# g1mv/density

Measured on AMD Instinct MI355X. Metric: MB/s encode+decode (round-trip) per GPU + compression ratio, dickens/enwik8, higher is better.
Workload: dtype u32

## Files before the change

### density_amd/csrc/api.hip

```cpp
#include "api_internal.hpp"

namespace density {
namespace api {

thread_local std::string g_last_error;
int g_profiling = 0;
int g_variant = 0;
uint64_t g_pass_decodes = 0;
uint64_t g_stream_stats[4] = {0, 0, 0, 0};
DeviceCtx g_ctx[kMaxDevices];

void set_error(const char* what, hipError_t e) {
    g_last_error = what;
    if (e != hipSuccess) { g_last_error += ": "; g_last_error += hipGetErrorString(e); }
}

DeviceCtx* acquire_ctx() {
    int dev = -1;
    hipError_t e = hipGetDevice(&dev);
    if (e != hipSuccess || dev < 0 || dev >= kMaxDevices) { set_error("no HIP device available", e); return nullptr; }
    DeviceCtx* c = &g_ctx[dev];
    std::lock_guard<std::mutex> lk(c->mu);
    if (!c->ready) {
        hipDeviceProp_t prop;
// ... 139 lines not shown
                         uint8_t* ws, hipStream_t s, density_hip_header_t* header_out, Form form) {
    const EncodePlan p = plan_encode(algo, n, chunk);
    if (p.n_chunks > 0xffffffffull) { set_error("too many chunks"); return DENSITY_HIP_ERR_ARGUMENT; }
    form = settle_form(form, algo, d_in, n, chunk, p.n_chunks);
    const size_t bound = form == Form::Paged ? container_bound_paged(algo, n, chunk) : form == Form::Slotted ? container_bound_slotted(algo, n, chunk) : container_bound(algo, n, chunk);
    if (cap < bound) { set_error("output capacity below density_hip_container_bound()"); return DENSITY_HIP_ERR_CAPACITY; }
    const uint32_t nch = (uint32_t)p.n_chunks;
    uint32_t* d_err = p.err(ws);
    uint64_t* d_sizes = p.sizes(ws);
    const density_hip_header_t hdr = make_header(algo, chunk, nch, n, (want_index(algo) ? DENSITY_HIP_FLAG_BLOCK_INDEX : 0) |
                                                 (form == Form::Slotted ? DENSITY_HIP_FLAG_SLOTTED : form == Form::Paged ? DENSITY_HIP_FLAG_PAGED : 0));
    const bool with_index = hdr.flags & DENSITY_HIP_FLAG_BLOCK_INDEX;
    const uint64_t pbase = payload_base(nch, n, with_index);
    uint8_t* d_index = with_index ? d_out + index_base(nch) : nullptr;
    Profiler prof(c, s);
    hipError_t e = hipMemsetAsync(d_err, 0, sizeof(uint32_t), s);
    if (e != hipSuccess) { set_error("hipMemsetAsync", e); return DENSITY_HIP_ERR_RUNTIME; }
    if (form == Form::Paged) {
        const uint64_t dir_base = paged_dir_base(nch, n), pages_base = paged_pages_base(nch, n, chunk);
        const uint32_t ppc = paged_pages_per_chunk(chunk);
        uint32_t* d_counter = p.page_counter(ws);
        e = hipMemsetAsync(d_counter, 0, sizeof(uint32_t), s);
        if (e == hipSuccess) e = launch_rotor_encode_paged(d_in, n, chunk, nch, d_out + pages_base, (uint32_t)std::min<uint64_t>((cap - pages_base) / kPageBytes, 0xffffu),
                                                         d_counter, reinterpret_cast<uint32_t*>(d_out + dir_base), page_dir_words(ppc), d_sizes, d_index, d_err, s);
        prof.mark(encode_kernel_name(algo));
        if (e == hipSuccess) e = launch_layout_encode_paged(d_sizes, nch, hdr, dir_base, dir_base + paged_dir_bytes(nch, chunk), pages_base, d_out, cap, d_counter, d_err, s);
        prof.mark("layout_encode");
    } else if (nch == 1 || form == Form::Slotted) {
        const uint64_t stride = nch == 1 ? 0 : p.stride;
        e = codec_encode(algo, d_in, n, chunk, nch, d_out + pbase, stride, d_sizes, d_index, p.tables(ws), p.zmap(ws), p.stage(ws), d_err, s);
        prof.mark(encode_kernel_name(algo));
        if (e == hipSuccess) e = launch_layout_encode(d_sizes, nch, hdr, pbase, d_out, cap, p.offsets(ws), d_err, s, stride);
        prof.mark("layout_encode");
    } else {
        constexpr uint32_t kStitchBatches = 4;
        uint32_t per = nch, batches = 1;
        if (algo == DENSITY_HIP_CHAMELEON && nch >= 512 && variant(kVarBatchedStitch)) {
            batches = nch / 256 < kStitchBatches ? nch / 256 : kStitchBatches;
            per = ((nch + batches - 1) / batches + 255) / 256 * 256;
            batches = (nch + per - 1) / per;
        }
        for (uint32_t k = 0; k < batches && e == hipSuccess; ++k) {
// ... 33 lines not shown
    const DecodePlan p = plan_decode(h.algo, h.n_chunks, h.chunk_size);
    uint32_t* d_err = p.err(ws);
    uint64_t *d_sizes = p.sizes(ws), *d_offsets = p.offsets(ws), *d_produced = p.produced(ws);
    uint32_t* d_zmap = p.zmap(ws);
    Profiler prof(c, s);
    hipError_t e = hipMemsetAsync(d_err, 0, sizeof(uint32_t), s);
    const bool with_index = h.flags & DENSITY_HIP_FLAG_BLOCK_INDEX;
    const uint8_t* d_index = with_index ? d_in + index_base(h.n_chunks) : nullptr;
    const size_t trailer = header_trailer(h), body_len = h.container_len - trailer;
    if (trailer) container_size = body_len;
    if (h.flags & DENSITY_HIP_FLAG_PAGED) {
        const size_t dir_base = paged_dir_base(h.n_chunks, h.total_len), pages_base = paged_pages_base(h.n_chunks, h.total_len, h.chunk_size);
        if (g_rotor_unsafe || !rotor_decode_eligible(d_out, h.n_chunks, h.chunk_size, h.total_len, d_index, d_zmap) || (uintptr_t)(d_in + pages_base) % 4 != 0) {
            set_error("a paged container needs the rotation decoder (chunks of at most 4 MiB, 4-byte aligned buffers)"); return DENSITY_HIP_ERR_UNSUPPORTED;
        }
        if (e == hipSuccess) e = launch_layout_decode_paged(d_in, h.n_chunks, d_sizes, d_offsets, s);
        prof.mark("layout_decode");
        if (e == hipSuccess) e = launch_rotor_decode_paged(d_in + pages_base, d_offsets, d_sizes, h.n_chunks, d_out, h.chunk_size, h.total_len, d_index,
                                                         reinterpret_cast<const uint32_t*>(d_in + dir_base), page_dir_words(paged_pages_per_chunk(h.chunk_size)),
                                                         (uint32_t)((body_len - pages_base) / kPageBytes), d_zmap, d_produced, d_err, s);
        prof.mark(decode_kernel_name(h.algo));
    } else {
        if (e == hipSuccess) e = launch_layout_decode(d_in, container_size, h.n_chunks, payload_base(h.n_chunks, h.total_len, with_index), d_sizes, d_offsets, d_err, s,
                                                      (h.flags & DENSITY_HIP_FLAG_SLOTTED) ? slot_stride(h.algo, h.chunk_size) : 0);
        prof.mark("layout_decode");
        if (e == hipSuccess) e = codec_decode(h.algo, d_in, d_offsets, d_sizes, h.n_chunks, d_out, h.chunk_size, h.total_len, true, d_index, d_produced, d_err, p.tables(ws), d_zmap, s,
                                              p.pass(ws, ws_size));
        prof.mark(decode_kernel_name(h.algo));
    }
    if (trailer) {
        if (e == hipSuccess) e = launch_checksum(d_out, h.total_len, h.chunk_size, h.n_chunks, reinterpret_cast<uint32_t*>(d_produced), d_in + body_len, d_err, s);
        prof.mark("checksum_verify");
    }
// ... 346 lines not shown
```

### density_amd/csrc/api_internal.hpp

```cpp
#pragma once
#include <hip/hip_runtime.h>

#include <algorithm>
#include <cstdio>
#include <cstring>
#include <initializer_list>
#include <mutex>
#include <string>
#include <vector>

#include "../../include/density_hip.h"
#include "kernels.hpp"

namespace density {
namespace api {

constexpr int kMaxDevices = 16;
constexpr size_t kAlign = 256;
constexpr size_t kMaxChunk = 1u << 30;

extern thread_local std::string g_last_error;
extern int g_profiling;
extern int g_variant;
extern uint64_t g_pass_decodes;
// ... 195 lines not shown
constexpr size_t kSerialTableBudget = 8ull << 30;
inline size_t serial_slots(int algo, size_t n_chunks) {
    if (algo == DENSITY_HIP_CHAMELEON) return 0;
    const size_t by_memory = kSerialTableBudget / serial_table_bytes(algo);
    size_t cap = kSerialSlots < by_memory ? kSerialSlots : by_memory;
    if (const char* e = debug_env("DENSITY_HIP_SERIAL_SLOTS")) { const size_t v = (size_t)atoll(e); if (v >= 1 && v < cap) cap = v; }
    return n_chunks < cap ? n_chunks : cap;
}
inline size_t serial_tables(int algo, size_t n_chunks) { return algo == DENSITY_HIP_CHAMELEON ? 0 : align_up(serial_slots(algo, n_chunks) * serial_table_bytes(algo), kAlign); }

inline size_t zmap_bytes(int algo, size_t n_chunks) { return (algo == DENSITY_HIP_CHAMELEON && n_chunks <= kMaxPipelinedChunks) ? align_up((n_chunks ? n_chunks : 1) * kZmapWordsPerChunk * 4, kAlign) : 0; }

struct EncodePlan {
    size_t chunk, n_chunks, stride, off_err, off_sizes, off_offsets, off_slots, off_tables, off_zmap, off_stage, total;
    uint32_t* err(uint8_t* ws) const { return reinterpret_cast<uint32_t*>(ws + off_err); }
    uint32_t* page_counter(uint8_t* ws) const { return err(ws) + 4; }
    uint64_t* sizes(uint8_t* ws) const { return reinterpret_cast<uint64_t*>(ws + off_sizes); }
    uint64_t* offsets(uint8_t* ws) const { return reinterpret_cast<uint64_t*>(ws + off_offsets); }
    uint64_t* carry(uint8_t* ws) const { return offsets(ws) + n_chunks; }
    uint8_t* slots(uint8_t* ws) const { return ws + off_slots; }
    uint8_t* tables(uint8_t* ws) const { return ws + off_tables; }
    uint32_t* zmap(uint8_t* ws) const { return off_stage > off_zmap ? reinterpret_cast<uint32_t*>(ws + off_zmap) : nullptr; }
    uint8_t* stage(uint8_t* ws) const { return total > off_stage ? ws + off_stage : nullptr; }
};
EncodePlan plan_encode(int algo, size_t n, size_t chunk);
struct DecodePlan {
    size_t off_err, off_sizes, off_offsets, off_produced, off_tables, off_zmap, off_pass, total, total_with_passes;
    uint32_t* err(uint8_t* ws) const { return reinterpret_cast<uint32_t*>(ws + off_err); }
    uint32_t* damaged(uint8_t* ws) const { return err(ws) + 1; }
    uint64_t* sizes(uint8_t* ws) const { return reinterpret_cast<uint64_t*>(ws + off_sizes); }
    uint64_t* offsets(uint8_t* ws) const { return reinterpret_cast<uint64_t*>(ws + off_offsets); }
// ... 40 lines not shown
```

### density_amd/csrc/container.hip

```cpp
#include "common.hpp"
#include "kernels.hpp"

namespace density {

namespace {

constexpr uint32_t kScanThreads = 1024;
constexpr uint32_t kHeaderBytes = 32;
static_assert(sizeof(density_hip_header_t) == kHeaderBytes, "container header is 32 bytes");

__device__ __forceinline__ uint64_t align16(uint64_t v) { return (v + 15ull) & ~15ull; }

__device__ __forceinline__ uint64_t block_inclusive_scan(uint64_t v, uint64_t* wave_sums , uint64_t* total) {
    const uint32_t lane = threadIdx.x & 63u, wave = threadIdx.x >> 6;
#pragma unroll
    for (int d = 1; d < 64; d <<= 1) {
        const uint32_t lo = bperm(lane >= (uint32_t)d ? lane - d : lane, (uint32_t)v);
        const uint32_t hi = bperm(lane >= (uint32_t)d ? lane - d : lane, (uint32_t)(v >> 32));
        if (lane >= (uint32_t)d) v += ((uint64_t)hi << 32) | lo;
    }
    if (lane == 63) wave_sums[wave] = v;
    __syncthreads();
    uint64_t prefix = 0, sum = 0;
    for (uint32_t i = 0; i < kScanThreads / 64; ++i) {
// ... 69 lines not shown
        *carry = end_scratch;
        if (is_last) {
            hdr.container_len = end_scratch;
            *reinterpret_cast<density_hip_header_t*>(container) = hdr;
        }
        if (end_scratch > capacity) atomicOr(err, 2u);
    }
    if (is_first) {
        const uint64_t table_end = kHeaderBytes + 4ull * hdr.n_chunks, ibase = (table_end + 15) / 16 * 16;
        const uint64_t iend = ibase + ((hdr.flags & DENSITY_HIP_FLAG_BLOCK_INDEX) ? (hdr.total_len + 255) / 256 : 0);
        if (threadIdx.x < ibase - table_end) container[table_end + threadIdx.x] = 0;
        if (threadIdx.x >= 32 && threadIdx.x - 32 < base - iend && base <= capacity) container[iend + threadIdx.x - 32] = 0;
    }
}

__global__ __launch_bounds__(kScanThreads) void layout_encode_paged_kernel(const uint64_t* __restrict__ sizes, uint32_t n, density_hip_header_t hdr, uint64_t dir_base,
                                                                           uint64_t dir_end, uint64_t pages_base, uint8_t* __restrict__ container, uint64_t capacity,
                                                                           const uint32_t* __restrict__ page_counter, uint32_t* __restrict__ err) {
    uint32_t* table = reinterpret_cast<uint32_t*>(container + kHeaderBytes);
    for (uint32_t i = threadIdx.x; i < n; i += kScanThreads) table[i] = (uint32_t)sizes[i];
    if (threadIdx.x == 0) {
        hdr.container_len = pages_base + (uint64_t)*page_counter * kPageBytes;
        *reinterpret_cast<density_hip_header_t*>(container) = hdr;
        if (hdr.container_len > capacity) atomicOr(err, 2u);
    }
    const uint64_t table_end = kHeaderBytes + 4ull * n, ibase = (table_end + 15) / 16 * 16;
    const uint64_t iend = ibase + (hdr.total_len + 255) / 256;
    if (threadIdx.x < ibase - table_end) container[table_end + threadIdx.x] = 0;
    if (threadIdx.x >= 32 && threadIdx.x - 32 < dir_base - iend) container[iend + threadIdx.x - 32] = 0;
    for (uint64_t i = dir_end + threadIdx.x; i < pages_base; i += kScanThreads) container[i] = 0;
}
__global__ __launch_bounds__(256) void clear_directory_tails_kernel(uint32_t n, uint64_t dir_base, uint64_t dir_end, uint8_t* __restrict__ container) {
    const uint32_t c = blockIdx.x * 4u + (threadIdx.x >> 6), lane = threadIdx.x & 63u;
    if (c >= n) return;
    const uint32_t words = (uint32_t)((dir_end - dir_base) / 4 / n);
    uint32_t* dir = reinterpret_cast<uint32_t*>(container + dir_base) + (uint64_t)c * words;
    const uint32_t used = dir[0];
    for (uint32_t w = 4u * (used + 1u) + lane; w < words; w += 64u) dir[w] = 0u;
}

__global__ __launch_bounds__(kScanThreads) void layout_decode_kernel(const uint8_t* __restrict__ container, uint64_t container_size,
                                                                     uint32_t n, uint64_t base, uint64_t* __restrict__ sizes,
                                                                     uint64_t* __restrict__ offsets, uint64_t* __restrict__ end_scratch,
                                                                     uint32_t* __restrict__ err, uint64_t slot_stride) {
    if (threadIdx.x == 0) *end_scratch = base;
    __syncthreads();
    layout_common<uint32_t>(reinterpret_cast<const uint32_t*>(container + kHeaderBytes), n, base, sizes, nullptr, offsets, end_scratch, container_size, err, slot_stride);
    __syncthreads();
    if (threadIdx.x == 0 && *end_scratch > container_size) atomicOr(err, 4u);
}

constexpr uint32_t kCopyThreads = 256;
constexpr uint32_t kCopyTile = kCopyThreads * 16u * 4u;

__global__ __launch_bounds__(kCopyThreads) void compact_kernel(const uint8_t* __restrict__ slots, uint64_t slot_stride,
// ... 52 lines not shown
    if (r3 != (56u + (lane & 7u))) bad |= 8u;
    __syncthreads();
    if (cells[200 + (lane & 7u)] != 156u + (lane & 7u)) bad |= 16u;
    if (bad) atomicOr(fail, bad);
}

}

hipError_t launch_layout_encode(const uint64_t* d_sizes, uint32_t n_chunks, density_hip_header_t hdr, uint64_t payload_base, uint8_t* d_container,
                                uint64_t capacity, uint64_t* d_offsets, uint32_t* d_err, hipStream_t stream, uint64_t slot_stride) {
    hipLaunchKernelGGL(layout_encode_kernel, dim3(1), dim3(kScanThreads), 0, stream, d_sizes, n_chunks, hdr, payload_base, d_container, capacity,
                       d_offsets, d_offsets + n_chunks, d_err, slot_stride);
    return hipGetLastError();
}

hipError_t launch_layout_encode_paged(const uint64_t* d_sizes, uint32_t n_chunks, density_hip_header_t hdr, uint64_t dir_base, uint64_t dir_end, uint64_t pages_base, uint8_t* d_container,
                                      uint64_t capacity, const uint32_t* d_page_counter, uint32_t* d_err, hipStream_t stream) {
    hipLaunchKernelGGL(layout_encode_paged_kernel, dim3(1), dim3(kScanThreads), 0, stream, d_sizes, n_chunks, hdr, dir_base, dir_end, pages_base, d_container, capacity, d_page_counter, d_err);
    if (n_chunks) hipLaunchKernelGGL(clear_directory_tails_kernel, dim3((n_chunks + 3) / 4), dim3(256), 0, stream, n_chunks, dir_base, dir_end, d_container);
    return hipGetLastError();
}

__global__ __launch_bounds__(kScanThreads) void layout_decode_paged_kernel(const uint8_t* __restrict__ container, uint32_t n, uint64_t* __restrict__ sizes, uint64_t* __restrict__ offsets) {
    const uint32_t* table = reinterpret_cast<const uint32_t*>(container + kHeaderBytes);
    for (uint32_t i = threadIdx.x; i < n; i += kScanThreads) { sizes[i] = table[i]; offsets[i] = 0; }
}
hipError_t launch_layout_decode_paged(const uint8_t* d_container, uint32_t n_chunks, uint64_t* d_sizes, uint64_t* d_offsets, hipStream_t stream) {
    hipLaunchKernelGGL(layout_decode_paged_kernel, dim3(1), dim3(kScanThreads), 0, stream, d_container, n_chunks, d_sizes, d_offsets);
    return hipGetLastError();
}

hipError_t launch_layout_encode_batch(const uint64_t* d_sizes, uint32_t first, uint32_t count, bool is_first, bool is_last, density_hip_header_t hdr,
                                      uint64_t payload_base, uint8_t* d_container, uint64_t capacity, uint64_t* d_offsets, uint64_t* d_carry, uint32_t* d_err,
                                      hipStream_t stream) {
    hipLaunchKernelGGL(layout_encode_batch_kernel, dim3(1), dim3(kScanThreads), 0, stream, d_sizes, first, count, is_first ? 1u : 0u, is_last ? 1u : 0u, hdr,
                       payload_base, d_container, capacity, d_offsets, d_carry, d_err);
    return hipGetLastError();
}

hipError_t launch_layout_decode(const uint8_t* d_container, uint64_t container_size, uint32_t n_chunks, uint64_t payload_base, uint64_t* d_sizes,
                                uint64_t* d_offsets, uint32_t* d_err, hipStream_t stream, uint64_t slot_stride) {
    hipLaunchKernelGGL(layout_decode_kernel, dim3(1), dim3(kScanThreads), 0, stream, d_container, container_size, n_chunks, payload_base, d_sizes,
                       d_offsets, d_offsets + n_chunks, d_err, slot_stride);
    return hipGetLastError();
}

// ... 18 lines not shown
```

### density_amd/csrc/kernels.hpp

```cpp
#pragma once
#include <hip/hip_runtime.h>
#include <stdint.h>
#include <stdlib.h>

#include "../../include/density_hip.h"

namespace density {

inline const char* debug_env(const char* name) {
#ifdef DENSITY_HIP_DEBUG
    return getenv(name);
#else
    (void)name;
    return nullptr;
#endif
}

extern bool g_force_simple;
hipError_t launch_chameleon_encode(const uint8_t* d_in, uint64_t total, uint64_t chunk_bytes, uint32_t n_chunks,
                                   uint8_t* d_out, uint64_t out_stride, uint64_t* d_sizes, uint8_t* d_index, uint32_t* d_zmap, uint32_t* d_err, hipStream_t stream);
hipError_t launch_chameleon_decode(const uint8_t* d_in, const uint64_t* d_offsets, const uint64_t* d_sizes,
                                   uint32_t n_chunks, uint8_t* d_out, uint64_t out_stride, uint64_t out_total,
                                   bool exact, const uint8_t* d_index, uint32_t* d_zmap, uint64_t* d_produced, uint32_t* d_err, hipStream_t stream);
constexpr uint32_t kZmapWordsPerChunk = 2048, kMaxPipelinedChunks = 16384;

constexpr uint32_t kPageShift = 16, kPageBytes = 1u << kPageShift;
__host__ __device__ inline uint32_t pages_per_chunk(uint64_t worst_stream_bytes) { return (uint32_t)(worst_stream_bytes / (kPageBytes - 4352u)) + 2u; }
__host__ __device__ inline uint32_t page_dir_words(uint32_t pages) { return 4u * (pages + 1u); }
constexpr uint64_t kPagedMaxChunk = 4ull << 20;
constexpr uint32_t kPagedMaxPages = 96;
bool rotor_encode_eligible(const uint8_t* d_in, uint64_t total, uint64_t chunk_bytes, uint32_t n_chunks);
hipError_t launch_rotor_encode_paged(const uint8_t* d_in, uint64_t total, uint64_t chunk_bytes, uint32_t n_chunks, uint8_t* d_pages, uint32_t page_limit,
                                     uint32_t* d_page_counter, uint32_t* d_dir, uint32_t dir_words, uint64_t* d_sizes, uint8_t* d_index, uint32_t* d_err, hipStream_t stream);
hipError_t launch_rotor_encode(const uint8_t* d_in, uint64_t total, uint64_t chunk_bytes, uint32_t n_chunks, uint8_t* d_out, uint64_t out_stride,
                               uint64_t* d_sizes, uint8_t* d_index, uint32_t* d_err, hipStream_t stream);
constexpr uint64_t kSegImageBytes = 128ull * 1024 + 8ull * 1024;
struct SegArgs {
    const uint8_t* init_images = nullptr;
    const uint32_t* init_guard = nullptr;
    uint8_t* final_images = nullptr;
    uint32_t* final_guard = nullptr;
    uint32_t* raw_blocks = nullptr;
    uint32_t* page_counter = nullptr;
    uint32_t* page_dir = nullptr;
    uint32_t page_dir_words = 0;
    uint32_t page_limit = 0;
    uint32_t lastwriters_only = 0;
};
hipError_t launch_rotor_encode_seg(const uint8_t* d_in, uint64_t total, uint64_t chunk_bytes, uint32_t n_chunks, uint8_t* d_out, uint64_t out_stride,
                                   uint64_t* d_sizes, uint32_t* d_err, SegArgs seg, hipStream_t stream);
hipError_t launch_rotor_lastwriters(const uint8_t* d_in, uint64_t chunk_bytes, uint32_t n_chunks, uint8_t* d_images, uint32_t* d_err, hipStream_t stream);
hipError_t launch_merge_images(const uint8_t* d_base, const uint8_t* d_lastwriters, uint8_t* d_start, uint32_t count, hipStream_t stream);
hipError_t launch_scan_offsets(const uint64_t* d_sizes, uint32_t first, uint32_t count, uint64_t* d_carry, uint64_t* d_offsets, hipStream_t stream);
hipError_t launch_compact_bytes(const uint8_t* d_src, uint64_t src_stride, const uint64_t* d_sizes, const uint64_t* d_offsets, uint32_t n_chunks,
                                uint8_t* d_dst, hipStream_t stream);
hipError_t launch_rotor_decode_seg(const uint8_t* d_in, const uint64_t* d_offsets, const uint64_t* d_sizes, uint32_t n_chunks, uint8_t* d_out,
                                   uint64_t out_stride, uint64_t out_total, const uint8_t* d_index, uint32_t* d_zmap, uint64_t* d_produced, uint32_t* d_err,
                                   SegArgs seg, hipStream_t stream);
bool rotor_decode_eligible(const uint8_t* d_out, uint32_t n_chunks, uint64_t out_stride, uint64_t out_total, const uint8_t* d_index, const uint32_t* d_zmap);
hipError_t launch_rotor_decode(const uint8_t* d_in, const uint64_t* d_offsets, const uint64_t* d_sizes, uint32_t n_chunks, uint8_t* d_out,
                               uint64_t out_stride, uint64_t out_total, bool exact, const uint8_t* d_index, uint32_t* d_zmap,
                               uint64_t* d_produced, uint32_t* d_err, hipStream_t stream);
// ... 32 lines not shown
extern int g_walk_blocks;
extern bool g_chain_walk;
bool decode_pass_eligible(int algo, const uint8_t* d_in, const uint8_t* d_out, uint32_t n_chunks, uint64_t out_stride, uint64_t out_total);
uint64_t decode_pass_scratch_bytes(uint64_t out_stride, uint32_t n_chunks);
hipError_t launch_decode_passes(int algo, const uint8_t* d_in, const uint64_t* d_offsets, const uint64_t* d_sizes, uint32_t n_chunks, uint8_t* d_out,
                                uint64_t out_stride, uint64_t out_total, bool exact, uint64_t* d_produced, uint32_t* d_err, uint8_t* d_scratch,
                                hipStream_t stream);

uint64_t stream_parse_workspace(uint64_t E);
hipError_t launch_stream_parse(const uint8_t* d_in, uint64_t E, uint64_t from_pos, uint8_t* d_ws, uint8_t* d_index, uint64_t index_cap, uint64_t* d_chunk_offset,
                               uint32_t chunk_blocks, uint32_t* d_pos32, uint32_t* d_info, hipStream_t stream);
hipError_t launch_seg_layout(const uint64_t* d_chunk_offset, uint32_t first, uint32_t count, uint64_t end, uint64_t* d_offsets, uint64_t* d_sizes, uint32_t* d_err, hipStream_t stream);

hipError_t launch_layout_encode(const uint64_t* d_sizes, uint32_t n_chunks, density_hip_header_t hdr, uint64_t payload_base, uint8_t* d_container,
                                uint64_t capacity, uint64_t* d_offsets, uint32_t* d_err, hipStream_t stream, uint64_t slot_stride = 0);
hipError_t launch_rotor_decode_paged(const uint8_t* d_pages, const uint64_t* d_offsets, const uint64_t* d_sizes, uint32_t n_chunks, uint8_t* d_out, uint64_t out_stride,
                                     uint64_t out_total, const uint8_t* d_index, const uint32_t* d_dir, uint32_t dir_words, uint32_t n_pages, uint32_t* d_zmap,
                                     uint64_t* d_produced, uint32_t* d_err, hipStream_t stream);
hipError_t launch_layout_encode_paged(const uint64_t* d_sizes, uint32_t n_chunks, density_hip_header_t hdr, uint64_t dir_base, uint64_t dir_end, uint64_t pages_base, uint8_t* d_container,
                                      uint64_t capacity, const uint32_t* d_page_counter, uint32_t* d_err, hipStream_t stream);
hipError_t launch_layout_decode_paged(const uint8_t* d_container, uint32_t n_chunks, uint64_t* d_sizes, uint64_t* d_offsets, hipStream_t stream);
hipError_t launch_layout_encode_batch(const uint64_t* d_sizes, uint32_t first, uint32_t count, bool is_first, bool is_last, density_hip_header_t hdr,
                                      uint64_t payload_base, uint8_t* d_container, uint64_t capacity, uint64_t* d_offsets, uint64_t* d_carry, uint32_t* d_err,
                                      hipStream_t stream);
hipError_t launch_layout_decode(const uint8_t* d_container, uint64_t container_size, uint32_t n_chunks, uint64_t payload_base,
                                uint64_t* d_sizes, uint64_t* d_offsets, uint32_t* d_err, hipStream_t stream, uint64_t slot_stride = 0);
hipError_t launch_compact(const uint8_t* d_slots, uint64_t slot_stride, const uint64_t* d_sizes, const uint64_t* d_offsets,
                          uint32_t n_chunks, uint8_t* d_container, const uint32_t* d_err, hipStream_t stream, bool more_follow = false);
hipError_t launch_selftest(uint32_t* d_fail, hipStream_t stream);

constexpr uint32_t kErrChecksum = 0x100u;
hipError_t launch_checksum(const uint8_t* d_data, uint64_t size, uint32_t chunk, uint32_t n_chunks, uint32_t* d_sums, const uint8_t* d_expect, uint32_t* d_err,
                           hipStream_t stream);
hipError_t launch_chunk_verdicts(const uint32_t* d_acc, uint64_t size, uint32_t chunk, uint32_t n_chunks, const uint8_t* d_expect, uint32_t* d_verdicts,
                                 uint32_t* d_count, uint32_t* d_err, hipStream_t stream);
hipError_t launch_blank_chunks(uint8_t* d_out, uint64_t size, uint32_t chunk, uint32_t n_chunks, const uint32_t* d_verdicts, hipStream_t stream);
// ... 6 lines not shown
```

### density_amd/csrc/rotor_decode.hip

```cpp
#include <cstdio>

#include "rotor_dev.hpp"

namespace density {

__device__ __forceinline__ bool index_fsm_consistent(const uint8_t* ix, uint32_t i, uint32_t nblk) {
    auto raw = [&](uint32_t b) -> bool { return (ix[b] & kIdxCopy) != 0; };
    auto inc = [&](uint32_t b) -> bool { return ix[b] <= 4u; };
    auto mult16 = [](uint32_t lo, uint32_t hi) -> uint32_t { return hi / 16u + 1u - (lo + 15u) / 16u; };
    auto halve = [](uint32_t s, uint32_t k) -> uint32_t { const uint32_t h = k < 32u ? s >> k : 0u; return s > 1u ? (h ? h : 1u) : s; };
    if (!raw(i)) {
        uint32_t u = i;
        while (u > 0 && raw(u - 1)) --u;
        const bool trigger = u > 0 && inc(u - 1);
        return !trigger || i + 1 >= nblk || raw(i + 1);
    }
    if (i > 0 && raw(i - 1)) return true;
    if (i == 0 || !inc(i - 1)) return false;
    const uint32_t t = i - 1;
    uint32_t u = t;
    while (u > 0 && raw(u - 1)) --u;
    if (u == 0 || !inc(u - 1)) return false;
    uint32_t L = 1;
    while (i + L < nblk && raw(i + L)) ++L;
// ... 19 lines not shown
    uint64_t* __restrict__ produced, uint32_t* __restrict__ err, SegArgs seg, uint64_t* __restrict__ prof) {
    constexpr int R = kDecRound, W = kDecWaves;
    constexpr uint32_t kThreads = W * 64, kScanThreads = 512, kPerThread = kRotMaxBlocks / kScanThreads;
    const uint32_t exact = flags & 1u, nap_far = (flags >> 8) & 15u, nap_near = (flags >> 16) & 15u;
    auto nap = [](uint32_t n) {
        if (n & 8u) __builtin_amdgcn_s_sleep(8);
        if (n & 4u) __builtin_amdgcn_s_sleep(4);
        if (n & 2u) __builtin_amdgcn_s_sleep(2);
        if (n & 1u) __builtin_amdgcn_s_sleep(1);
    };

    const uint32_t lane = threadIdx.x & 63u;
    const uint32_t wave = rfl(threadIdx.x >> 6);
    const uint64_t chunk = blockIdx.x;
    PhaseClock<kProf> clk(blockIdx.x == 0 ? prof : nullptr);
    const uint8_t* src = in + offsets[chunk];
    const uint8_t* idx = index + chunk * (out_stride / kBlock);
    const uint64_t elen64 = sizes[chunk];
    uint8_t* dst = out + chunk * out_stride;
    const uint64_t room_all = out_total - chunk * out_stride;
    const uint64_t cap = room_all < out_stride ? room_all : out_stride;
    const uint32_t elen = elen64 > 0xfff00000ull ? 0xfff00000u : (uint32_t)elen64;
    const uint32_t nblk = (uint32_t)((cap + kBlock - 1) / kBlock);
    constexpr uint32_t dSync = kDecSync;
    const ZmapLds zmap{kDecZmap};
    const uint32_t sy = dSync;

    {
        uint4* p = reinterpret_cast<uint4*>(smem);
        const uint4 z = make_uint4(0, 0, 0, 0);
        const uint4* image = seg.init_images ? reinterpret_cast<const uint4*>(seg.init_images + chunk * kSegImageBytes) : nullptr;
        for (uint32_t i = threadIdx.x; i < kTableBytes / 16; i += kThreads) p[i] = image ? image[i] : z;
        for (uint32_t i = threadIdx.x; i < kZmapBytes / 16; i += kThreads) reinterpret_cast<uint4*>(smem + kDecZmap)[i] = image ? image[kTableBytes / 16 + i] : z;
// ... 413 lines not shown
    if ((uintptr_t)d_index % 4 != 0 || (n_chunks > 1 && (out_stride / kBlock) % 4 != 0)) return false;
    return (uintptr_t)d_out % 4 == 0 && (n_chunks == 1 || out_stride % 4 == 0);
}
hipError_t launch_rotor_decode(const uint8_t* d_in, const uint64_t* d_offsets, const uint64_t* d_sizes, uint32_t n_chunks, uint8_t* d_out,
                               uint64_t out_stride, uint64_t out_total, bool exact, const uint8_t* d_index, uint32_t* d_zmap,
                               uint64_t* d_produced, uint32_t* d_err, hipStream_t stream) {
    uint64_t* prof = rot_prof_buffer();
    auto kernel = prof ? chameleon_decode_rot<true> : chameleon_decode_rot<false>;
    hipError_t e = hipFuncSetAttribute((const void*)kernel, hipFuncAttributeMaxDynamicSharedMemorySize, (int)kDecLds);
    if (e != hipSuccess) return e;
    hipLaunchKernelGGL(kernel, dim3(n_chunks), dim3(kDecThreads), kDecLds, stream, d_in, d_offsets, d_sizes, d_out, out_stride, out_total,
                       (exact ? 1u : 0u) | decode_naps(), d_index, d_zmap, d_produced, d_err, SegArgs{}, prof);
    rot_prof_report("decode", "stage A | stage B | operands | D wait | exchange | quads | Z chain | stores", prof, stream, kDecWaves);
    return hipGetLastError();
}
hipError_t launch_rotor_decode_paged(const uint8_t* d_pages, const uint64_t* d_offsets, const uint64_t* d_sizes, uint32_t n_chunks, uint8_t* d_out, uint64_t out_stride,
                                     uint64_t out_total, const uint8_t* d_index, const uint32_t* d_dir, uint32_t dir_words, uint32_t n_pages, uint32_t* d_zmap,
                                     uint64_t* d_produced, uint32_t* d_err, hipStream_t stream) {
    auto kernel = chameleon_decode_rot<false, true>;
    hipError_t e = hipFuncSetAttribute((const void*)kernel, hipFuncAttributeMaxDynamicSharedMemorySize, (int)kDecLdsPaged);
    if (e != hipSuccess) return e;
    SegArgs pg;
    pg.page_dir = const_cast<uint32_t*>(d_dir); pg.page_dir_words = dir_words; pg.page_limit = n_pages;
    hipLaunchKernelGGL(kernel, dim3(n_chunks), dim3(kDecThreads), kDecLdsPaged, stream, d_pages, d_offsets, d_sizes, d_out, out_stride, out_total,
                       1u | decode_naps(), d_index, d_zmap, d_produced, d_err, pg, (uint64_t*)nullptr);
    return hipGetLastError();
}
hipError_t launch_rotor_decode_seg(const uint8_t* d_in, const uint64_t* d_offsets, const uint64_t* d_sizes, uint32_t n_chunks, uint8_t* d_out,
                                   uint64_t out_stride, uint64_t out_total, const uint8_t* d_index, uint32_t* d_zmap, uint64_t* d_produced, uint32_t* d_err,
                                   SegArgs seg, hipStream_t stream) {
    auto kernel = chameleon_decode_rot<false>;
    hipError_t e = hipFuncSetAttribute((const void*)kernel, hipFuncAttributeMaxDynamicSharedMemorySize, (int)kDecLds);
    if (e != hipSuccess) return e;
    hipLaunchKernelGGL(kernel, dim3(n_chunks), dim3(kDecThreads), kDecLds, stream, d_in, d_offsets, d_sizes, d_out, out_stride, out_total, decode_naps(),
                       d_index, d_zmap, d_produced, d_err, seg, (uint64_t*)nullptr);
    return hipGetLastError();
}

}
// ... 1 lines not shown
```

### density_amd/csrc/rotor_encode.hip

```cpp
#include "rotor_dev.hpp"

namespace density {

namespace {

#define DENSITY_ROT_PF16 \
    "global_load_dword v240, %0, off offset:0\n\t" \
    "global_load_dword v241, %0, off offset:256\n\t" \
    "global_load_dword v242, %0, off offset:512\n\t" \
    "global_load_dword v243, %0, off offset:768\n\t" \
    "global_load_dword v244, %0, off offset:1024\n\t" \
    "global_load_dword v245, %0, off offset:1280\n\t" \
    "global_load_dword v246, %0, off offset:1536\n\t" \
    "global_load_dword v247, %0, off offset:1792\n\t" \
    "global_load_dword v248, %0, off offset:2048\n\t" \
    "global_load_dword v249, %0, off offset:2304\n\t" \
    "global_load_dword v250, %0, off offset:2560\n\t" \
    "global_load_dword v251, %0, off offset:2816\n\t" \
    "global_load_dword v252, %0, off offset:3072\n\t" \
    "global_load_dword v253, %0, off offset:3328\n\t" \
    "global_load_dword v254, %0, off offset:3584\n\t" \
    "global_load_dword v255, %0, off offset:3840\n\t"
#define DENSITY_ROT_MV16 \
    "v_mov_b32 %0, v240\n\t" \
// ... 6 lines not shown
    "v_mov_b32 %7, v247\n\t" \
    "v_mov_b32 %8, v248\n\t" \
    "v_mov_b32 %9, v249\n\t" \
    "v_mov_b32 %10, v250\n\t" \
    "v_mov_b32 %11, v251\n\t" \
    "v_mov_b32 %12, v252\n\t" \
    "v_mov_b32 %13, v253\n\t" \
    "v_mov_b32 %14, v254\n\t" \
    "v_mov_b32 %15, v255\n\t"
#define DENSITY_ROT_STAGE16 "v240", "v241", "v242", "v243", "v244", "v245", "v246", "v247", "v248", "v249", "v250", "v251", "v252", "v253", "v254", "v255"
__device__ __forceinline__ void prefetch_quads(const uint8_t* p) { asm volatile(DENSITY_ROT_PF16 : : "v"(p) : "memory", DENSITY_ROT_STAGE16); }
template <bool kDrained>
__device__ __forceinline__ void quads_landed(uint32_t (&q)[16]) {
    if constexpr (kDrained) asm volatile("s_waitcnt vmcnt(0)\n\t" DENSITY_ROT_MV16 : DENSITY_ROT_EACH16("=v", q) : : DENSITY_ROT_STAGE16);
    else asm volatile("s_waitcnt vmcnt(16)\n\t" DENSITY_ROT_MV16 : DENSITY_ROT_EACH16("=v", q) : : DENSITY_ROT_STAGE16);
}

}

template <bool kProf, bool PAGED = false, bool SPLIT = false>
__global__ __launch_bounds__(SPLIT ? 2 * kEncWaves * 64 : kEncWaves * 64) void chameleon_encode_rot(
    const uint8_t* __restrict__ in, uint64_t total, uint64_t chunk_bytes, uint8_t* __restrict__ out, uint64_t out_stride,
    uint64_t* __restrict__ sizes, uint8_t* __restrict__ index, uint32_t* __restrict__ err, SegArgs seg, uint64_t* __restrict__ prof) {
    constexpr int R = kEncRound, W = kEncWaves;
    constexpr uint32_t kThreads = SPLIT ? 2u * W * 64u : W * 64u;
    const uint32_t lane = threadIdx.x & 63u;
    const uint32_t wave = rfl(threadIdx.x >> 6);
    const uint64_t chunk = blockIdx.x;
    PhaseClock<kProf> clk(blockIdx.x == 0 ? prof : nullptr);
    const uint8_t* src = in + chunk * chunk_bytes;
// ... 701 lines not shown
            block_in_order(g, qv, a, m, vv, sg, raw);
            emit_block(dst + opos, qv, sg, raw);
            const uint32_t nh = (uint32_t)__builtin_popcountll(sg);
            if (idx && lane == 0) idx[b] = (uint8_t)(raw ? kIdxCopy : nh);
            if (seg.raw_blocks && raw && lane == 0) atomicAdd(seg.raw_blocks + chunk, 1u);
            opos += raw ? kBlock : kSig + kBlock - 2u * nh;
        }
        if (seg.final_guard && lane == 0) seg.final_guard[chunk] = pack_guard(g) | (g.penalty == 0 ? 0x80000000u : 0u);
        const uint64_t end = encode_ragged_block(src, len, nfull, dst, opos, g, idx, 0u, zmap, lane);
        if (PAGED) {
            const u32x4 st = lds_peek4(sy + kSyPage);
            const uint32_t base = rfl(st.x), before = rfl(st.y), count = rfl(st.w);
            if (lane == 0) {
                dir[4u * count + 2u] = (uint32_t)end - base;
                *reinterpret_cast<uint4*>(dir) = make_uint4(count, 0u, 0u, 0u);
                sizes[chunk] = (uint64_t)before + ((uint32_t)end - base);
            }
        } else
        if (lane == 0) sizes[chunk] = end;
    }
    if (seg.final_images) {
        wg_barrier();
        uint4* image = reinterpret_cast<uint4*>(seg.final_images + chunk * kSegImageBytes);
        const uint4* p = reinterpret_cast<const uint4*>(smem);
        for (uint32_t i = threadIdx.x; i < (kTableBytes + kZmapBytes) / 16; i += kThreads) image[i] = p[i];
    }
}

__global__ __launch_bounds__(1024) void chameleon_lastwriters_rot(const uint8_t* __restrict__ in, uint64_t chunk_bytes, uint8_t* __restrict__ images,
                                                                   uint32_t* __restrict__ err) {
    constexpr int R = 16, W = 16;
    const uint32_t lane = threadIdx.x & 63u;
// ... 82 lines not shown
    auto kernel = split ? (prof ? chameleon_encode_rot<true, false, true> : chameleon_encode_rot<false, false, true>)
                        : (prof ? chameleon_encode_rot<true> : chameleon_encode_rot<false>);
    hipError_t e = hipFuncSetAttribute((const void*)kernel, hipFuncAttributeMaxDynamicSharedMemorySize, (int)enc_lds());
    if (e != hipSuccess) return e;
    hipLaunchKernelGGL(kernel, dim3(n_chunks), dim3(enc_threads()), enc_lds(), stream, d_in, total, chunk_bytes, d_out, out_stride, d_sizes, d_index,
                       d_err, SegArgs{}, prof);
    if (split)
        rot_prof_report("encode (split)",
                        "chain waves 0-7: hash | D wait | exchange | signatures | O wait+commit | ring: wait for the quads | post | ring: the reads "
                        "(+ in-order rounds);  emit waves 8-15: - | ring transfer incl. the wait for the slot | - | - | mail box wait | - | emit | -",
                        prof, stream, 2 * kEncWaves);
    else
        rot_prof_report("encode", "hash | D wait | exchange | signatures | O wait+commit | load wait | emit | in-order rounds", prof, stream, kEncWaves);
    return hipGetLastError();
}
hipError_t launch_rotor_encode_paged(const uint8_t* d_in, uint64_t total, uint64_t chunk_bytes, uint32_t n_chunks, uint8_t* d_pages, uint32_t page_limit,
                                     uint32_t* d_page_counter, uint32_t* d_dir, uint32_t dir_words, uint64_t* d_sizes, uint8_t* d_index, uint32_t* d_err,
                                     hipStream_t stream) {
    auto kernel = g_rotor_split ? chameleon_encode_rot<false, true, true> : chameleon_encode_rot<false, true>;
    hipError_t e = hipFuncSetAttribute((const void*)kernel, hipFuncAttributeMaxDynamicSharedMemorySize, (int)enc_lds());
    if (e != hipSuccess) return e;
    SegArgs pg;
    pg.page_counter = d_page_counter; pg.page_dir = d_dir; pg.page_dir_words = dir_words; pg.page_limit = page_limit;
    hipLaunchKernelGGL(kernel, dim3(n_chunks), dim3(enc_threads()), enc_lds(), stream, d_in, total, chunk_bytes, d_pages, (uint64_t)0, d_sizes, d_index,
                       d_err, pg, (uint64_t*)nullptr);
    return hipGetLastError();
}
hipError_t launch_rotor_encode_seg(const uint8_t* d_in, uint64_t total, uint64_t chunk_bytes, uint32_t n_chunks, uint8_t* d_out, uint64_t out_stride,
                                   uint64_t* d_sizes, uint32_t* d_err, SegArgs seg, hipStream_t stream) {
    auto kernel = g_rotor_split ? chameleon_encode_rot<false, false, true> : chameleon_encode_rot<false>;
    hipError_t e = hipFuncSetAttribute((const void*)kernel, hipFuncAttributeMaxDynamicSharedMemorySize, (int)enc_lds());
    if (e != hipSuccess) return e;
    hipLaunchKernelGGL(kernel, dim3(n_chunks), dim3(enc_threads()), enc_lds(), stream, d_in, total, chunk_bytes, d_out, out_stride, d_sizes,
                       (uint8_t*)nullptr, d_err, seg, (uint64_t*)nullptr);
    return hipGetLastError();
}
hipError_t launch_rotor_lastwriters(const uint8_t* d_in, uint64_t chunk_bytes, uint32_t n_chunks, uint8_t* d_images, uint32_t* d_err, hipStream_t stream) {
    if (n_chunks == 0) return hipSuccess;
// ... 15 lines not shown
```

Before: 1.270 million.

## Fold paged layout kernels into the rotor encode and decode kernels

The paged encode no longer launches separate layout and directory-tail clearing kernels. The last block to finish, found through an atomic done-counter, writes the header, the size table and the padding, and each block clears its own directory tail. The paged decode reads the 32-bit size table straight from the container instead of running a layout_decode kernel, and the two workspace memsets become one. This removes several small kernel launches and their serialization per round trip, at the cost of a last-block-arrives pattern that relies on memory ordering. It also hardcodes header fields (algo, flags) inside the kernel.

```diff
diff --git a/density_amd/csrc/api.hip b/density_amd/csrc/api.hip
--- a/density_amd/csrc/api.hip
+++ b/density_amd/csrc/api.hip
@@ -177,18 +177,14 @@
     const uint64_t pbase = payload_base(nch, n, with_index);
     uint8_t* d_index = with_index ? d_out + index_base(nch) : nullptr;
     Profiler prof(c, s);
-    hipError_t e = hipMemsetAsync(d_err, 0, sizeof(uint32_t), s);
+    hipError_t e = hipMemsetAsync(d_err, 0, form == Form::Paged ? EncodePlan::kPagedClearBytes : sizeof(uint32_t), s);
     if (e != hipSuccess) { set_error("hipMemsetAsync", e); return DENSITY_HIP_ERR_RUNTIME; }
     if (form == Form::Paged) {
         const uint64_t dir_base = paged_dir_base(nch, n), pages_base = paged_pages_base(nch, n, chunk);
         const uint32_t ppc = paged_pages_per_chunk(chunk);
-        uint32_t* d_counter = p.page_counter(ws);
-        e = hipMemsetAsync(d_counter, 0, sizeof(uint32_t), s);
-        if (e == hipSuccess) e = launch_rotor_encode_paged(d_in, n, chunk, nch, d_out + pages_base, (uint32_t)std::min<uint64_t>((cap - pages_base) / kPageBytes, 0xffffu),
-                                                         d_counter, reinterpret_cast<uint32_t*>(d_out + dir_base), page_dir_words(ppc), d_sizes, d_index, d_err, s);
+        e = launch_rotor_encode_paged(d_in, n, chunk, nch, d_out, d_out + pages_base, (uint32_t)std::min<uint64_t>((cap - pages_base) / kPageBytes, 0xffffu),
+                                      p.paged_counters(ws), reinterpret_cast<uint32_t*>(d_out + dir_base), page_dir_words(ppc), d_sizes, d_index, d_err, s);
         prof.mark(encode_kernel_name(algo));
-        if (e == hipSuccess) e = launch_layout_encode_paged(d_sizes, nch, hdr, dir_base, dir_base + paged_dir_bytes(nch, chunk), pages_base, d_out, cap, d_counter, d_err, s);
-        prof.mark("layout_encode");
     } else if (nch == 1 || form == Form::Slotted) {
         const uint64_t stride = nch == 1 ? 0 : p.stride;
         e = codec_encode(algo, d_in, n, chunk, nch, d_out + pbase, stride, d_sizes, d_index, p.tables(ws), p.zmap(ws), p.stage(ws), d_err, s);
@@ -252,9 +248,8 @@
         if (g_rotor_unsafe || !rotor_decode_eligible(d_out, h.n_chunks, h.chunk_size, h.total_len, d_index, d_zmap) || (uintptr_t)(d_in + pages_base) % 4 != 0) {
             set_error("a paged container needs the rotation decoder (chunks of at most 4 MiB, 4-byte aligned buffers)"); return DENSITY_HIP_ERR_UNSUPPORTED;
         }
-        if (e == hipSuccess) e = launch_layout_decode_paged(d_in, h.n_chunks, d_sizes, d_offsets, s);
         prof.mark("layout_decode");
-        if (e == hipSuccess) e = launch_rotor_decode_paged(d_in + pages_base, d_offsets, d_sizes, h.n_chunks, d_out, h.chunk_size, h.total_len, d_index,
+        if (e == hipSuccess) e = launch_rotor_decode_paged(d_in + pages_base, reinterpret_cast<const uint32_t*>(d_in + sizeof(density_hip_header_t)), h.n_chunks, d_out, h.chunk_size, h.total_len, d_index,
                                                          reinterpret_cast<const uint32_t*>(d_in + dir_base), page_dir_words(paged_pages_per_chunk(h.chunk_size)),
                                                          (uint32_t)((body_len - pages_base) / kPageBytes), d_zmap, d_produced, d_err, s);
         prof.mark(decode_kernel_name(h.algo));
diff --git a/density_amd/csrc/api_internal.hpp b/density_amd/csrc/api_internal.hpp
--- a/density_amd/csrc/api_internal.hpp
+++ b/density_amd/csrc/api_internal.hpp
@@ -233,7 +233,8 @@
 struct EncodePlan {
     size_t chunk, n_chunks, stride, off_err, off_sizes, off_offsets, off_slots, off_tables, off_zmap, off_stage, total;
     uint32_t* err(uint8_t* ws) const { return reinterpret_cast<uint32_t*>(ws + off_err); }
-    uint32_t* page_counter(uint8_t* ws) const { return err(ws) + 4; }
+    uint32_t* paged_counters(uint8_t* ws) const { return err(ws) + 4; }
+    static constexpr size_t kPagedClearBytes = 32;
     uint64_t* sizes(uint8_t* ws) const { return reinterpret_cast<uint64_t*>(ws + off_sizes); }
     uint64_t* offsets(uint8_t* ws) const { return reinterpret_cast<uint64_t*>(ws + off_offsets); }
     uint64_t* carry(uint8_t* ws) const { return offsets(ws) + n_chunks; }
diff --git a/density_amd/csrc/container.hip b/density_amd/csrc/container.hip
--- a/density_amd/csrc/container.hip
+++ b/density_amd/csrc/container.hip
@@ -107,31 +107,6 @@
     }
 }
 
-__global__ __launch_bounds__(kScanThreads) void layout_encode_paged_kernel(const uint64_t* __restrict__ sizes, uint32_t n, density_hip_header_t hdr, uint64_t dir_base,
-                                                                           uint64_t dir_end, uint64_t pages_base, uint8_t* __restrict__ container, uint64_t capacity,
-                                                                           const uint32_t* __restrict__ page_counter, uint32_t* __restrict__ err) {
-    uint32_t* table = reinterpret_cast<uint32_t*>(container + kHeaderBytes);
-    for (uint32_t i = threadIdx.x; i < n; i += kScanThreads) table[i] = (uint32_t)sizes[i];
-    if (threadIdx.x == 0) {
-        hdr.container_len = pages_base + (uint64_t)*page_counter * kPageBytes;
-        *reinterpret_cast<density_hip_header_t*>(container) = hdr;
-        if (hdr.container_len > capacity) atomicOr(err, 2u);
-    }
-    const uint64_t table_end = kHeaderBytes + 4ull * n, ibase = (table_end + 15) / 16 * 16;
-    const uint64_t iend = ibase + (hdr.total_len + 255) / 256;
-    if (threadIdx.x < ibase - table_end) container[table_end + threadIdx.x] = 0;
-    if (threadIdx.x >= 32 && threadIdx.x - 32 < dir_base - iend) container[iend + threadIdx.x - 32] = 0;
-    for (uint64_t i = dir_end + threadIdx.x; i < pages_base; i += kScanThreads) container[i] = 0;
-}
-__global__ __launch_bounds__(256) void clear_directory_tails_kernel(uint32_t n, uint64_t dir_base, uint64_t dir_end, uint8_t* __restrict__ container) {
-    const uint32_t c = blockIdx.x * 4u + (threadIdx.x >> 6), lane = threadIdx.x & 63u;
-    if (c >= n) return;
-    const uint32_t words = (uint32_t)((dir_end - dir_base) / 4 / n);
-    uint32_t* dir = reinterpret_cast<uint32_t*>(container + dir_base) + (uint64_t)c * words;
-    const uint32_t used = dir[0];
-    for (uint32_t w = 4u * (used + 1u) + lane; w < words; w += 64u) dir[w] = 0u;
-}
-
 __global__ __launch_bounds__(kScanThreads) void layout_decode_kernel(const uint8_t* __restrict__ container, uint64_t container_size,
                                                                      uint32_t n, uint64_t base, uint64_t* __restrict__ sizes,
                                                                      uint64_t* __restrict__ offsets, uint64_t* __restrict__ end_scratch,
@@ -214,22 +189,6 @@
     return hipGetLastError();
 }
 
-hipError_t launch_layout_encode_paged(const uint64_t* d_sizes, uint32_t n_chunks, density_hip_header_t hdr, uint64_t dir_base, uint64_t dir_end, uint64_t pages_base, uint8_t* d_container,
-                                      uint64_t capacity, const uint32_t* d_page_counter, uint32_t* d_err, hipStream_t stream) {
-    hipLaunchKernelGGL(layout_encode_paged_kernel, dim3(1), dim3(kScanThreads), 0, stream, d_sizes, n_chunks, hdr, dir_base, dir_end, pages_base, d_container, capacity, d_page_counter, d_err);
-    if (n_chunks) hipLaunchKernelGGL(clear_directory_tails_kernel, dim3((n_chunks + 3) / 4), dim3(256), 0, stream, n_chunks, dir_base, dir_end, d_container);
-    return hipGetLastError();
-}
-
-__global__ __launch_bounds__(kScanThreads) void layout_decode_paged_kernel(const uint8_t* __restrict__ container, uint32_t n, uint64_t* __restrict__ sizes, uint64_t* __restrict__ offsets) {
-    const uint32_t* table = reinterpret_cast<const uint32_t*>(container + kHeaderBytes);
-    for (uint32_t i = threadIdx.x; i < n; i += kScanThreads) { sizes[i] = table[i]; offsets[i] = 0; }
-}
-hipError_t launch_layout_decode_paged(const uint8_t* d_container, uint32_t n_chunks, uint64_t* d_sizes, uint64_t* d_offsets, hipStream_t stream) {
-    hipLaunchKernelGGL(layout_decode_paged_kernel, dim3(1), dim3(kScanThreads), 0, stream, d_container, n_chunks, d_sizes, d_offsets);
-    return hipGetLastError();
-}
-
 hipError_t launch_layout_encode_batch(const uint64_t* d_sizes, uint32_t first, uint32_t count, bool is_first, bool is_last, density_hip_header_t hdr,
                                       uint64_t payload_base, uint8_t* d_container, uint64_t capacity, uint64_t* d_offsets, uint64_t* d_carry, uint32_t* d_err,
                                       hipStream_t stream) {
diff --git a/density_amd/csrc/kernels.hpp b/density_amd/csrc/kernels.hpp
--- a/density_amd/csrc/kernels.hpp
+++ b/density_amd/csrc/kernels.hpp
@@ -30,8 +30,8 @@
 constexpr uint64_t kPagedMaxChunk = 4ull << 20;
 constexpr uint32_t kPagedMaxPages = 96;
 bool rotor_encode_eligible(const uint8_t* d_in, uint64_t total, uint64_t chunk_bytes, uint32_t n_chunks);
-hipError_t launch_rotor_encode_paged(const uint8_t* d_in, uint64_t total, uint64_t chunk_bytes, uint32_t n_chunks, uint8_t* d_pages, uint32_t page_limit,
-                                     uint32_t* d_page_counter, uint32_t* d_dir, uint32_t dir_words, uint64_t* d_sizes, uint8_t* d_index, uint32_t* d_err, hipStream_t stream);
+hipError_t launch_rotor_encode_paged(const uint8_t* d_in, uint64_t total, uint64_t chunk_bytes, uint32_t n_chunks, uint8_t* d_container, uint8_t* d_pages, uint32_t page_limit,
+                                     uint32_t* d_counters, uint32_t* d_dir, uint32_t dir_words, uint64_t* d_sizes, uint8_t* d_index, uint32_t* d_err, hipStream_t stream);
 hipError_t launch_rotor_encode(const uint8_t* d_in, uint64_t total, uint64_t chunk_bytes, uint32_t n_chunks, uint8_t* d_out, uint64_t out_stride,
                                uint64_t* d_sizes, uint8_t* d_index, uint32_t* d_err, hipStream_t stream);
 constexpr uint64_t kSegImageBytes = 128ull * 1024 + 8ull * 1024;
@@ -46,6 +46,9 @@
     uint32_t page_dir_words = 0;
     uint32_t page_limit = 0;
     uint32_t lastwriters_only = 0;
+    const uint32_t* size_table = nullptr;
+    uint8_t* container = nullptr;
+    uint32_t* done_counter = nullptr;
 };
 hipError_t launch_rotor_encode_seg(const uint8_t* d_in, uint64_t total, uint64_t chunk_bytes, uint32_t n_chunks, uint8_t* d_out, uint64_t out_stride,
                                    uint64_t* d_sizes, uint32_t* d_err, SegArgs seg, hipStream_t stream);
@@ -108,12 +111,9 @@
 
 hipError_t launch_layout_encode(const uint64_t* d_sizes, uint32_t n_chunks, density_hip_header_t hdr, uint64_t payload_base, uint8_t* d_container,
                                 uint64_t capacity, uint64_t* d_offsets, uint32_t* d_err, hipStream_t stream, uint64_t slot_stride = 0);
-hipError_t launch_rotor_decode_paged(const uint8_t* d_pages, const uint64_t* d_offsets, const uint64_t* d_sizes, uint32_t n_chunks, uint8_t* d_out, uint64_t out_stride,
+hipError_t launch_rotor_decode_paged(const uint8_t* d_pages, const uint32_t* d_size_table, uint32_t n_chunks, uint8_t* d_out, uint64_t out_stride,
                                      uint64_t out_total, const uint8_t* d_index, const uint32_t* d_dir, uint32_t dir_words, uint32_t n_pages, uint32_t* d_zmap,
                                      uint64_t* d_produced, uint32_t* d_err, hipStream_t stream);
-hipError_t launch_layout_encode_paged(const uint64_t* d_sizes, uint32_t n_chunks, density_hip_header_t hdr, uint64_t dir_base, uint64_t dir_end, uint64_t pages_base, uint8_t* d_container,
-                                      uint64_t capacity, const uint32_t* d_page_counter, uint32_t* d_err, hipStream_t stream);
-hipError_t launch_layout_decode_paged(const uint8_t* d_container, uint32_t n_chunks, uint64_t* d_sizes, uint64_t* d_offsets, hipStream_t stream);
 hipError_t launch_layout_encode_batch(const uint64_t* d_sizes, uint32_t first, uint32_t count, bool is_first, bool is_last, density_hip_header_t hdr,
                                       uint64_t payload_base, uint8_t* d_container, uint64_t capacity, uint64_t* d_offsets, uint64_t* d_carry, uint32_t* d_err,
                                       hipStream_t stream);
diff --git a/density_amd/csrc/rotor_decode.hip b/density_amd/csrc/rotor_decode.hip
--- a/density_amd/csrc/rotor_decode.hip
+++ b/density_amd/csrc/rotor_decode.hip
@@ -57,9 +57,9 @@
     const uint32_t wave = rfl(threadIdx.x >> 6);
     const uint64_t chunk = blockIdx.x;
     PhaseClock<kProf> clk(blockIdx.x == 0 ? prof : nullptr);
-    const uint8_t* src = in + offsets[chunk];
+    const uint8_t* src = PAGED ? in : in + offsets[chunk];
     const uint8_t* idx = index + chunk * (out_stride / kBlock);
-    const uint64_t elen64 = sizes[chunk];
+    const uint64_t elen64 = PAGED ? (uint64_t)seg.size_table[chunk] : sizes[chunk];
     uint8_t* dst = out + chunk * out_stride;
     const uint64_t room_all = out_total - chunk * out_stride;
     const uint64_t cap = room_all < out_stride ? room_all : out_stride;
@@ -503,15 +503,15 @@
     rot_prof_report("decode", "stage A | stage B | operands | D wait | exchange | quads | Z chain | stores", prof, stream, kDecWaves);
     return hipGetLastError();
 }
-hipError_t launch_rotor_decode_paged(const uint8_t* d_pages, const uint64_t* d_offsets, const uint64_t* d_sizes, uint32_t n_chunks, uint8_t* d_out, uint64_t out_stride,
+hipError_t launch_rotor_decode_paged(const uint8_t* d_pages, const uint32_t* d_size_table, uint32_t n_chunks, uint8_t* d_out, uint64_t out_stride,
                                      uint64_t out_total, const uint8_t* d_index, const uint32_t* d_dir, uint32_t dir_words, uint32_t n_pages, uint32_t* d_zmap,
                                      uint64_t* d_produced, uint32_t* d_err, hipStream_t stream) {
     auto kernel = chameleon_decode_rot<false, true>;
     hipError_t e = hipFuncSetAttribute((const void*)kernel, hipFuncAttributeMaxDynamicSharedMemorySize, (int)kDecLdsPaged);
     if (e != hipSuccess) return e;
     SegArgs pg;
-    pg.page_dir = const_cast<uint32_t*>(d_dir); pg.page_dir_words = dir_words; pg.page_limit = n_pages;
-    hipLaunchKernelGGL(kernel, dim3(n_chunks), dim3(kDecThreads), kDecLdsPaged, stream, d_pages, d_offsets, d_sizes, d_out, out_stride, out_total,
+    pg.page_dir = const_cast<uint32_t*>(d_dir); pg.page_dir_words = dir_words; pg.page_limit = n_pages; pg.size_table = d_size_table;
+    hipLaunchKernelGGL(kernel, dim3(n_chunks), dim3(kDecThreads), kDecLdsPaged, stream, d_pages, (const uint64_t*)nullptr, (const uint64_t*)nullptr, d_out, out_stride, out_total,
                        1u | decode_naps(), d_index, d_zmap, d_produced, d_err, pg, (uint64_t*)nullptr);
     return hipGetLastError();
 }
diff --git a/density_amd/csrc/rotor_encode.hip b/density_amd/csrc/rotor_encode.hip
--- a/density_amd/csrc/rotor_encode.hip
+++ b/density_amd/csrc/rotor_encode.hip
@@ -44,6 +44,29 @@
 __device__ __forceinline__ void quads_landed(uint32_t (&q)[16]) {
     if constexpr (kDrained) asm volatile("s_waitcnt vmcnt(0)\n\t" DENSITY_ROT_MV16 : DENSITY_ROT_EACH16("=v", q) : : DENSITY_ROT_STAGE16);
     else asm volatile("s_waitcnt vmcnt(16)\n\t" DENSITY_ROT_MV16 : DENSITY_ROT_EACH16("=v", q) : : DENSITY_ROT_STAGE16);
+}
+
+
+__device__ __forceinline__ void paged_front_matter(uint8_t* __restrict__ container, uint64_t* sizes, uint32_t n, uint64_t total, uint64_t chunk_bytes,
+                                                   uint32_t* page_counter, uint32_t page_limit, uint32_t dir_words, uint32_t* err, uint32_t lane) {
+    constexpr uint64_t kHeaderBytes = sizeof(density_hip_header_t);
+    static_assert(kHeaderBytes == 32 && offsetof(density_hip_header_t, chunk_size) == 8 && offsetof(density_hip_header_t, total_len) == 16, "the header as the two stores below write it");
+    const uint64_t table_end = kHeaderBytes + 4ull * n, ibase = (table_end + 15) / 16 * 16;
+    const uint64_t iend = ibase + (total + 255) / 256, dir_base = (iend + 15) / 16 * 16;
+    const uint64_t dir_end = dir_base + 4ull * dir_words * n, pages_base = (dir_end + 255) / 256 * 256;
+    uint32_t* table = reinterpret_cast<uint32_t*>(container + kHeaderBytes);
+    for (uint32_t i = lane; i < n; i += 64u) table[i] = (uint32_t)__hip_atomic_load(sizes + i, __ATOMIC_RELAXED, __HIP_MEMORY_SCOPE_AGENT);
+    if (lane == 0) {
+        const uint32_t pages = __hip_atomic_load(page_counter, __ATOMIC_RELAXED, __HIP_MEMORY_SCOPE_AGENT);
+        const uint64_t container_len = pages_base + (uint64_t)pages * kPageBytes;
+        const uint32_t word1 = (uint32_t)DENSITY_HIP_CHAMELEON | (1u << 8) | ((uint32_t)(DENSITY_HIP_FLAG_BLOCK_INDEX | DENSITY_HIP_FLAG_PAGED) << 16);
+        reinterpret_cast<uint4*>(container)[0] = make_uint4(DENSITY_HIP_MAGIC, word1, (uint32_t)chunk_bytes, n);
+        reinterpret_cast<uint4*>(container)[1] = make_uint4((uint32_t)total, (uint32_t)(total >> 32), (uint32_t)container_len, (uint32_t)(container_len >> 32));
+        if (pages > page_limit) atomicOr(err, 2u);
+    }
+    if (lane < ibase - table_end) container[table_end + lane] = 0;
+    if (lane < dir_base - iend) container[iend + lane] = 0;
+    for (uint64_t i = dir_end + lane; i < pages_base; i += 64u) container[i] = 0;
 }
 
 }
@@ -775,8 +798,13 @@
             if (lane == 0) {
                 dir[4u * count + 2u] = (uint32_t)end - base;
                 *reinterpret_cast<uint4*>(dir) = make_uint4(count, 0u, 0u, 0u);
-                sizes[chunk] = (uint64_t)before + ((uint32_t)end - base);
-            }
+                __hip_atomic_store(sizes + chunk, (uint64_t)before + ((uint32_t)end - base), __ATOMIC_RELAXED, __HIP_MEMORY_SCOPE_AGENT);
+            }
+            for (uint32_t w = 4u * (count + 1u) + lane; w < seg.page_dir_words; w += 64u) dir[w] = 0u;
+            asm volatile("s_waitcnt vmcnt(0)" ::: "memory");
+            const uint32_t arrived = rfl(lane == 0 ? __hip_atomic_fetch_add(seg.done_counter, 1u, __ATOMIC_RELAXED, __HIP_MEMORY_SCOPE_AGENT) : 0u);
+            if (arrived == gridDim.x - 1u)
+                paged_front_matter(seg.container, sizes, gridDim.x, total, chunk_bytes, seg.page_counter, seg.page_limit, seg.page_dir_words, err, lane);
         } else
         if (lane == 0) sizes[chunk] = end;
     }
@@ -889,14 +917,14 @@
         rot_prof_report("encode", "hash | D wait | exchange | signatures | O wait+commit | load wait | emit | in-order rounds", prof, stream, kEncWaves);
     return hipGetLastError();
 }
-hipError_t launch_rotor_encode_paged(const uint8_t* d_in, uint64_t total, uint64_t chunk_bytes, uint32_t n_chunks, uint8_t* d_pages, uint32_t page_limit,
-                                     uint32_t* d_page_counter, uint32_t* d_dir, uint32_t dir_words, uint64_t* d_sizes, uint8_t* d_index, uint32_t* d_err,
+hipError_t launch_rotor_encode_paged(const uint8_t* d_in, uint64_t total, uint64_t chunk_bytes, uint32_t n_chunks, uint8_t* d_container, uint8_t* d_pages, uint32_t page_limit,
+                                     uint32_t* d_counters, uint32_t* d_dir, uint32_t dir_words, uint64_t* d_sizes, uint8_t* d_index, uint32_t* d_err,
                                      hipStream_t stream) {
     auto kernel = g_rotor_split ? chameleon_encode_rot<false, true, true> : chameleon_encode_rot<false, true>;
     hipError_t e = hipFuncSetAttribute((const void*)kernel, hipFuncAttributeMaxDynamicSharedMemorySize, (int)enc_lds());
     if (e != hipSuccess) return e;
     SegArgs pg;
-    pg.page_counter = d_page_counter; pg.page_dir = d_dir; pg.page_dir_words = dir_words; pg.page_limit = page_limit;
+    pg.page_counter = d_counters; pg.done_counter = d_counters + 1; pg.page_dir = d_dir; pg.page_dir_words = dir_words; pg.page_limit = page_limit; pg.container = d_container;
     hipLaunchKernelGGL(kernel, dim3(n_chunks), dim3(enc_threads()), enc_lds(), stream, d_in, total, chunk_bytes, d_pages, (uint64_t)0, d_sizes, d_index,
                        d_err, pg, (uint64_t*)nullptr);
     return hipGetLastError();
```

Result: faster. 1.284 million (median of 6 runs) (+1.1%).
